# tum-vision/mem

Measured on AMD Instinct MI355X. Metric: pretrain samples/sec (ViT-B, 224^2 event voxels), higher is better.
Workload: dtype bf16; 1 GPU; MEM pretrain ViT-Base/16, 224^2 2-bin event voxels, bf16, batch 256 per GPU (BASELINE configs[1]); step = rasterize 256x30k events + event_norm + masks + ViT fwd/CE/bwd + clip + AdamW; global_batch=256, parallelism=dp1, stochastic_depth=work skipping, optimizer=AdamW as one launch in front of the next forward, last_block_mlp_rows=rows that reach the head

## Files before the change

mem_amd/csrc/misc.hip:

```cpp
#include "common.h"

namespace {

using namespace memhip;

typedef __attribute__((ext_vector_type(4))) __bf16 bf16x4;
typedef __attribute__((ext_vector_type(8))) __bf16 bf16x8;

__global__ __launch_bounds__(256) void cast_kernel(const float* __restrict__ in, __bf16* __restrict__ out,
                                                   long long n4) {
  for (long long i = (long long)blockIdx.x * 256 + threadIdx.x; i < n4; i += (long long)gridDim.x * 256) {
    const float4 v = reinterpret_cast<const float4*>(in)[i];
    bf16x4 o;
    o[0] = (__bf16)v.x; o[1] = (__bf16)v.y; o[2] = (__bf16)v.z; o[3] = (__bf16)v.w;
    reinterpret_cast<bf16x4*>(out)[i] = o;
  }
}

template <typename IN>
__global__ __launch_bounds__(256) void transpose_kernel(const IN* __restrict__ in, long long ldin, int R,
                                                        int Cc, __bf16* __restrict__ out, long long ldout,
                                                        int R_pad, float* __restrict__ cs0, int c0b, int c0e,
                                                        float* __restrict__ cs1, int c1b, int c1e) {
  __shared__ __bf16 tile[64][66];
  const int r0 = blockIdx.x * 64, c0 = blockIdx.y * 64;
  const int t = threadIdx.x;
#pragma unroll
  for (int pass = 0; pass < 2; ++pass) {
    const int rl = (t >> 3) + pass * 32, cl = (t & 7) * 8;
    const int r = r0 + rl;
#pragma unroll
    for (int k = 0; k < 8; ++k) {
      const int c = c0 + cl + k;
      __bf16 v = (__bf16)0.f;
      if (r < R && c < Cc) v = (__bf16)(float)in[(long long)r * ldin + c];
      tile[rl][cl + k] = v;
    }
  }
  __syncthreads();
#pragma unroll
  for (int pass = 0; pass < 2; ++pass) {
    const int cl = (t >> 3) + pass * 32, rl = (t & 7) * 8;
    const int c = c0 + cl;
    bf16x8 o;
    float s = 0.f;
#pragma unroll
    for (int k = 0; k < 8; ++k) { o[k] = tile[rl + k][cl]; s += (float)o[k]; }
    if (c < Cc && r0 + rl < R_pad)
      *reinterpret_cast<bf16x8*>(out + (long long)c * ldout + r0 + rl) = o;
    if (cs0 || cs1) {
      s += __shfl_xor(s, 1); s += __shfl_xor(s, 2); s += __shfl_xor(s, 4);
      if ((t & 7) == 0 && c < Cc) {
        if (cs0 && c >= c0b && c < c0e) atomicAdd(cs0 + (c - c0b), s);
        if (cs1 && c >= c1b && c < c1e) atomicAdd(cs1 + (c - c1b), s);
      }
    }
  }
}

struct TransposeDesc { const float* in; long long ldin; long long R; long long Cc; __bf16* out; long long ldout; };
__global__ __launch_bounds__(256) void transpose_cast_batched_kernel(const TransposeDesc* __restrict__ desc,
                                                                     const int* __restrict__ tile_prefix, int n) {
  __shared__ __bf16 tile[64][66];
  int mi = 0;
  while (mi + 1 < n && (int)blockIdx.x >= tile_prefix[mi + 1]) ++mi;
  const TransposeDesc d = desc[mi];
  const int local = blockIdx.x - tile_prefix[mi];
  const int R = (int)d.R, Cc = (int)d.Cc;
  const int tr = (R + 63) / 64;
  const int r0 = (local % tr) * 64, c0 = (local / tr) * 64;
  const int t = threadIdx.x;
  const int R_pad = (int)(d.ldout < (long long)tr * 64 ? d.ldout : (long long)tr * 64);
#pragma unroll
  for (int pass = 0; pass < 2; ++pass) {
    const int rl = (t >> 3) + pass * 32, cl = (t & 7) * 8;
    const int r = r0 + rl, c = c0 + cl;
    const float* src = d.in + (long long)r * d.ldin + c;
    if (r < R && c + 8 <= Cc && ((d.ldin & 3) == 0) && (((unsigned long long)d.in & 15) == 0)) {
      const float4 a = reinterpret_cast<const float4*>(src)[0], b = reinterpret_cast<const float4*>(src)[1];
      const float v[8] = {a.x, a.y, a.z, a.w, b.x, b.y, b.z, b.w};
#pragma unroll
      for (int k = 0; k < 8; ++k) tile[rl][cl + k] = (__bf16)v[k];
    } else {
#pragma unroll
      for (int k = 0; k < 8; ++k) tile[rl][cl + k] = (r < R && c + k < Cc) ? (__bf16)src[k] : (__bf16)0.f;
    }
  }
  __syncthreads();
#pragma unroll
  for (int pass = 0; pass < 2; ++pass) {
    const int cl = (t >> 3) + pass * 32, rl = (t & 7) * 8;
    const int c = c0 + cl;
    bf16x8 o;
#pragma unroll
    for (int k = 0; k < 8; ++k) o[k] = tile[rl + k][cl];
    if (c < Cc && r0 + rl < R_pad) *reinterpret_cast<bf16x8*>(d.out + (long long)c * d.ldout + r0 + rl) = o;
  }
}

__global__ __launch_bounds__(256) void im2col_kernel(const float* __restrict__ x, int B, int C, int H, int W,
                                                     int ph, int pw, __bf16* __restrict__ out) {
  const int gw = W / pw, gh = H / ph;
  const int K = C * ph * pw, K8 = K >> 3;
  const long long total = (long long)B * gh * gw * K8;
  for (long long i = (long long)blockIdx.x * 256 + threadIdx.x; i < total; i += (long long)gridDim.x * 256) {
    const int k8 = (int)(i % K8);
    const long long row = i / K8;
    const int k = k8 * 8;
    const int c = k / (ph * pw), rem = k - c * ph * pw, py = rem / pw, px = rem - py * pw;
    const int gx = (int)(row % gw);
    const long long t = row / gw;
    const int gy = (int)(t % gh), b = (int)(t / gh);
    const float* src = x + (((long long)b * C + c) * H + gy * ph + py) * W + gx * pw + px;
    const float4 a = reinterpret_cast<const float4*>(src)[0], d = reinterpret_cast<const float4*>(src)[1];
    bf16x8 o;
    o[0] = (__bf16)a.x; o[1] = (__bf16)a.y; o[2] = (__bf16)a.z; o[3] = (__bf16)a.w;
    o[4] = (__bf16)d.x; o[5] = (__bf16)d.y; o[6] = (__bf16)d.z; o[7] = (__bf16)d.w;
    reinterpret_cast<bf16x8*>(out)[i] = o;
  }
}

__global__ __launch_bounds__(256) void fill_cls_kernel(float* __restrict__ x, long long ldx, int B, int T, int D,
                                                       const float* __restrict__ cls) {
  const int b = blockIdx.x;
  for (int c = threadIdx.x; c < D; c += 256) x[(long long)b * T * ldx + c] = cls[c];
}

__global__ __launch_bounds__(256) void relpos_gather_kernel(const float* __restrict__ table,
                                                            const int* __restrict__ idx, int T, int TP, int Hh,
                                                            float* __restrict__ bias, float* __restrict__ biasT) {
  const long long total = (long long)Hh * TP * TP;
  for (long long i = (long long)blockIdx.x * 256 + threadIdx.x; i < total; i += (long long)gridDim.x * 256) {
    const int k = (int)(i % TP);
    const long long t = i / TP;
    const int q = (int)(t % TP), h = (int)(t / TP);
    float v = 0.f;
    if (q < T && k < T) v = table[(long long)idx[q * T + k] * Hh + h];
    bias[i] = v;
    if (biasT) biasT[((long long)h * TP + k) * TP + q] = v;
  }
}


__global__ __launch_bounds__(256) void gemv_acc_kernel(const __bf16* __restrict__ W, long long ldw, int N, int K,
                                                       const float* __restrict__ x, float* __restrict__ y,
                                                       float* __restrict__ x_acc, float* __restrict__ zero) {
  const int lane = threadIdx.x & 63;
  const int n = blockIdx.x * 4 + (threadIdx.x >> 6);
  if (n < N) {
    float s = 0.f;
    for (int k = lane * 8; k < K; k += 512) {
      const bf16x8 w = *reinterpret_cast<const bf16x8*>(W + (long long)n * ldw + k);
      const float4 a = *reinterpret_cast<const float4*>(x + k), b = *reinterpret_cast<const float4*>(x + k + 4);
      s += (float)w[0] * a.x + (float)w[1] * a.y + (float)w[2] * a.z + (float)w[3] * a.w + (float)w[4] * b.x +
           (float)w[5] * b.y + (float)w[6] * b.z + (float)w[7] * b.w;
    }
    for (int o = 32; o > 0; o >>= 1) s += __shfl_xor(s, o);
    if (lane == 0) y[n] += s;
  }
  if (blockIdx.x == 0) {
    for (int k = threadIdx.x; k < K; k += blockDim.x) {
      if (x_acc) x_acc[k] += x[k];
      if (zero) zero[k] = 0.f;
    }
  }
}

}

extern "C" int memhip_cast_f32_bf16(const float* in, void* out, int64_t n, memhip_stream_t stream) {
  MEMHIP_REQUIRE(n >= 0 && n % 4 == 0, "cast: n must be a multiple of 4");
  if (n == 0) return MEMHIP_OK;
  MEMHIP_REQUIRE(in && out, "cast: null pointer");
  const long long n4 = n / 4;
  int blocks = (int)((n4 + 255) / 256);
  if (blocks > 4096) blocks = 4096;
  hipLaunchKernelGGL(cast_kernel, dim3(blocks), dim3(256), 0, as_stream(stream), in, (__bf16*)out, n4);
  return check_launch("cast_f32_bf16");
}

extern "C" int memhip_transpose_cast_f32_bf16(const float* in, int64_t ldin, int R, int Cc, void* out,
                                              int64_t ldout, memhip_stream_t stream) {
  MEMHIP_REQUIRE(R > 0 && Cc > 0 && in && out, "transpose_cast: bad arguments");
  MEMHIP_REQUIRE(ldout % 8 == 0 && ldout >= R, "transpose_cast: ldout");
  const int R_pad = (int)(ldout < (int64_t)cdiv(R, 64) * 64 ? ldout : (int64_t)cdiv(R, 64) * 64);
  hipLaunchKernelGGL(transpose_kernel<float>, dim3(cdiv(R, 64), cdiv(Cc, 64)), dim3(256), 0, as_stream(stream), in,
                     (long long)ldin, R, Cc, (__bf16*)out, (long long)ldout, R_pad, (float*)nullptr, 0, 0,
                     (float*)nullptr, 0, 0);
  return check_launch("transpose_cast");
}

extern "C" int memhip_transpose_cast_batched(const void* desc, const int32_t* tile_prefix, int n, int total_tiles,
                                             memhip_stream_t stream) {
  MEMHIP_REQUIRE(n >= 0 && total_tiles >= 0, "transpose_cast_batched: bad arguments");
  if (n == 0 || total_tiles == 0) return MEMHIP_OK;
  MEMHIP_REQUIRE(desc && tile_prefix, "transpose_cast_batched: null pointer");
  static_assert(sizeof(TransposeDesc) == 48, "descriptor = 6 x 8 bytes");
  hipLaunchKernelGGL(transpose_cast_batched_kernel, dim3(total_tiles), dim3(256), 0, as_stream(stream),
                     (const TransposeDesc*)desc, tile_prefix, n);
  return check_launch("transpose_cast_batched");
}

extern "C" int memhip_transpose_bf16(const void* in, int64_t ldin, int R, int Cc, void* out, int64_t ldout,
                                     int R_pad, float* colsum0, int c0_begin, int c0_end, float* colsum1,
                                     int c1_begin, int c1_end, memhip_stream_t stream) {
  MEMHIP_REQUIRE(R >= 0 && Cc > 0 && in && out, "transpose: bad arguments");
  MEMHIP_REQUIRE(R_pad >= R && R_pad % 64 == 0 && ldout >= R_pad && ldout % 8 == 0,
                 "transpose: R_pad=%d must be a multiple of 64 and <= ldout", R_pad);
  if (R_pad == 0) return MEMHIP_OK;
  hipLaunchKernelGGL(transpose_kernel<__bf16>, dim3(R_pad / 64, cdiv(Cc, 64)), dim3(256), 0, as_stream(stream),
                     (const __bf16*)in, (long long)ldin, R, Cc, (__bf16*)out, (long long)ldout, R_pad, colsum0,
                     c0_begin, c0_end, colsum1, c1_begin, c1_end);
  return check_launch("transpose_bf16");
}

extern "C" int memhip_im2col_bf16(const float* x, int B, int C, int H, int W, int ph, int pw, void* out,
                                  memhip_stream_t stream) {
  MEMHIP_REQUIRE(B >= 0 && C > 0 && ph > 0 && pw > 0 && H % ph == 0 && W % pw == 0, "im2col: bad shape");
  MEMHIP_REQUIRE(pw % 8 == 0 && W % 4 == 0, "im2col: patch width must be a multiple of 8");
  if (B == 0) return MEMHIP_OK;
  MEMHIP_REQUIRE(x && out, "im2col: null pointer");
  const long long total = (long long)B * (H / ph) * (W / pw) * (C * ph * pw / 8);
  int blocks = (int)((total + 255) / 256);
  if (blocks > 8192) blocks = 8192;
  hipLaunchKernelGGL(im2col_kernel, dim3(blocks), dim3(256), 0, as_stream(stream), x, B, C, H, W, ph, pw,
                     (__bf16*)out);
  return check_launch("im2col");
}

__global__ __launch_bounds__(256) void copy_samples_kernel(const float* __restrict__ src, float* __restrict__ dst,
                                                           const int* __restrict__ ids, long long n_per_sample) {
  const long long base = (long long)ids[blockIdx.y] * n_per_sample;
  const float4* s4 = reinterpret_cast<const float4*>(src + base);
  float4* d4 = reinterpret_cast<float4*>(dst + base);
  for (long long i = (long long)blockIdx.x * 256 + threadIdx.x; i < n_per_sample / 4; i += (long long)gridDim.x * 256) d4[i] = s4[i];
}

extern "C" int memhip_copy_samples_f32(const float* src, float* dst, const int32_t* ids, int n, int64_t n_per_sample,
// ... 136 lines not shown
```

mem_amd/csrc/rowops.hip:

```cpp
#include "common.h"
#include "dropout.hpp"

#include <type_traits>

namespace {

using namespace memhip;

typedef __attribute__((ext_vector_type(4))) __bf16 bf16x4;
typedef __attribute__((ext_vector_type(8))) __bf16 bf16x8;

__device__ __forceinline__ float wsum(float v) {
  for (int o = 32; o > 0; o >>= 1) v += __shfl_xor(v, o);
  return v;
}
__device__ __forceinline__ float wmax(float v) {
  for (int o = 32; o > 0; o >>= 1) v = fmaxf(v, __shfl_xor(v, o));
  return v;
}

__device__ __forceinline__ float div_newton(float a, float b, float r) {
  const float q0 = a * r;
  return fmaf(fmaf(-q0, b, a), r, q0);
}

constexpr int kMaxChunks = 8;

template <bool FULL>
__device__ __forceinline__ bool chunk_ok(int i, int nch) {
  if constexpr (FULL) return true;
  else return i < nch;
}

__device__ __forceinline__ int wave_id() { return __builtin_amdgcn_readfirstlane((int)(threadIdx.x >> 6)); }

struct RowWalk {
  int r, smp, off, stride, q, rem, rps;
  __device__ __forceinline__ RowWalk(int r0, int stride_, int rps_) : r(r0), stride(stride_), rps(rps_) {
    smp = r0 / rps; off = r0 - smp * rps;
    q = stride / rps; rem = stride - q * rps;
  }
  __device__ __forceinline__ void next() {
    r += stride; smp += q; off += rem;
    if (off >= rps) { off -= rps; ++smp; }
  }
};

__device__ __forceinline__ void stage_columns(float4* dst, const float* a, const float* b, int nch) {
  for (int i = threadIdx.x; i < nch; i += 256) {
    dst[i] = reinterpret_cast<const float4*>(a)[i];
    dst[nch + i] = b ? reinterpret_cast<const float4*>(b)[i] : float4{1.f, 1.f, 1.f, 1.f};
  }
  __syncthreads();
}

__device__ __forceinline__ int opaque(int v) {
  asm volatile("" : "+v"(v));
  return v;
}

__device__ __forceinline__ float mul_rn(float a, float b) {
#pragma clang fp contract(off)
  return a * b;
}
__device__ __forceinline__ float sub_rn(float a, float b) {
#pragma clang fp contract(off)
  return a - b;
}
__device__ __forceinline__ float ln_dx(float gg, float xh, float m1, float m2) { return __fmaf_rn(-xh, m2, sub_rn(gg, m1)); }
__device__ __forceinline__ float sq2(float a, float b) { return __fmaf_rn(a, a, mul_rn(b, b)); }

template <int NCH, bool FULL>
__global__ __launch_bounds__(256) void ln_fwd_kernel(const float* __restrict__ x, long long ldx,
                                                     const int* __restrict__ row_idx, int R, int D,
                                                     const float* __restrict__ gamma,
                                                     const float* __restrict__ beta, float eps,
                                                     __bf16* __restrict__ y, long long ldy,
                                                     float* __restrict__ mean, float* __restrict__ rstd) {
  extern __shared__ float red[];
  const int lane = threadIdx.x & 63;
  const int r0 = blockIdx.x * 4 + wave_id();
  const bool act = r0 < R;
  const int r = act ? r0 : R - 1;
  const long long src = row_idx ? row_idx[r] : r;
  const float4* xr = reinterpret_cast<const float4*>(x + src * ldx);
  const int nch = D >> 2;
  float4 v[NCH];
#pragma unroll
  for (int c = 0; c < NCH; ++c) {
    const int i = lane + c * 64;
    if (chunk_ok<FULL>(i, nch)) v[c] = xr[i];
  }
  constexpr int NST = (64 * NCH + 255) / 256;
  float4 sg[NST], sb[NST];
#pragma unroll
  for (int k = 0; k < NST; ++k) {
    const int i = min((int)threadIdx.x + k * 256, nch - 1);
    sg[k] = reinterpret_cast<const float4*>(gamma)[i];
    sb[k] = reinterpret_cast<const float4*>(beta)[i];
  }
  __builtin_amdgcn_sched_barrier(0);
  float s = 0.f;
#pragma unroll
  for (int c = 0; c < NCH; ++c)
    if (chunk_ok<FULL>(lane + c * 64, nch)) s += (v[c].x + v[c].y) + (v[c].z + v[c].w);
  const float mu = wsum(s) / (float)D;
  float4* lgb = reinterpret_cast<float4*>(red);
#pragma unroll
  for (int k = 0; k < NST; ++k) {
    const int i = min((int)threadIdx.x + k * 256, nch - 1);
    lgb[i] = sg[k];
    lgb[nch + i] = sb[k];
  }
  float q = 0.f;
#pragma unroll
  for (int c = 0; c < NCH; ++c) {
    if (chunk_ok<FULL>(lane + c * 64, nch)) {
      const float a = v[c].x - mu, b = v[c].y - mu, cc = v[c].z - mu, d = v[c].w - mu;
      q += sq2(a, b) + sq2(cc, d);
    }
  }
  const float var = wsum(q) / (float)D;
  const float rs = 1.0f / sqrtf(var + eps);
  __syncthreads();
  if (!act) return;
  if (lane == 0) { mean[r] = mu; rstd[r] = rs; }
  bf16x4* yr = reinterpret_cast<bf16x4*>(y + (long long)r * ldy);
#pragma unroll
  for (int c = 0; c < NCH; ++c) {
    const int i = lane + c * 64;
    if (chunk_ok<FULL>(i, nch)) {
      const float4 g = lgb[i], b = lgb[nch + i];
      bf16x4 o;
      o[0] = (__bf16)__fmaf_rn(mul_rn(v[c].x - mu, rs), g.x, b.x);
      o[1] = (__bf16)__fmaf_rn(mul_rn(v[c].y - mu, rs), g.y, b.y);
      o[2] = (__bf16)__fmaf_rn(mul_rn(v[c].z - mu, rs), g.z, b.z);
      o[3] = (__bf16)__fmaf_rn(mul_rn(v[c].w - mu, rs), g.w, b.w);
      yr[i] = o;
    }
  }
}

__device__ __forceinline__ void vm_drain() { __builtin_amdgcn_s_waitcnt(0x0F70); }

template <int NCH, bool FULL, bool ACC>
__global__ __launch_bounds__(256) void ln_bwd_kernel(const __bf16* __restrict__ dy, long long lddy,
                                                     const float* __restrict__ x, long long ldx,
                                                     const int* __restrict__ row_idx, int R, int D,
                                                     const float* __restrict__ gamma,
                                                     const float* __restrict__ mean,
                                                     const float* __restrict__ rstd,
                                                     float* __restrict__ dres, long long lddres,
                                                     float* __restrict__ dgamma, float* __restrict__ dbeta) {
  extern __shared__ float red[];
  const int lane = threadIdx.x & 63, wave = wave_id();
  const int nch = D >> 2;
  float4 ag[NCH], ab[NCH];
#pragma unroll
  for (int c = 0; c < NCH; ++c) {
    ag[c] = float4{0, 0, 0, 0};
    ab[c] = float4{0, 0, 0, 0};
  }
  const int rstride = gridDim.x * 4;
  float4 xn[NCH], prev[NCH];
  bf16x4 dn[NCH];
  auto issue = [&](int r, long long src, int lane) {
    const float4* xr = reinterpret_cast<const float4*>(x + src * ldx);
    const bf16x4* dyr = reinterpret_cast<const bf16x4*>(dy + (long long)r * lddy);
#pragma unroll
    for (int c = 0; c < NCH; ++c) {
      const int i = lane + c * 64;
      if (chunk_ok<FULL>(i, nch)) {
        xn[c] = xr[i];
        dn[c] = dyr[i];
      }
    }
  };
  auto issue_prev = [&](long long src, int lane) {
    const float4* o = reinterpret_cast<const float4*>(dres + src * lddres);
#pragma unroll
    for (int c = 0; c < NCH; ++c) {
      const int i = lane + c * 64;
      if (chunk_ok<FULL>(i, nch)) prev[c] = o[i];
    }
  };
  int r = blockIdx.x * 4 + wave;
  long long src = 0;
  float mu = 0.f, rs = 0.f;
  if (r < R) {
    src = row_idx ? row_idx[r] : r;
    issue(r, src, lane);
    if constexpr (ACC) issue_prev(src, lane);
    mu = mean[r]; rs = rstd[r];
  }
  float4* lg = reinterpret_cast<float4*>(red);
  for (int i = threadIdx.x; i < nch; i += 256) lg[i] = reinterpret_cast<const float4*>(gamma)[i];
  __syncthreads();
  int r1 = r + rstride;
  long long src1 = 0;
  if (r1 < R) src1 = row_idx ? row_idx[r1] : r1;
  int r2 = r1 + rstride;
  vm_drain();
  while (r < R) {
    float4 xh[NCH], gg[NCH];
    float s1 = 0.f, s2 = 0.f;
    const int ol = opaque(lane);
    const float4* lgl = lg + ol;
#pragma unroll
    for (int c = 0; c < NCH; ++c) {
      const int i = lane + c * 64;
      if (chunk_ok<FULL>(i, nch)) {
        const float4 xv = xn[c];
        const bf16x4 d4 = dn[c];
        const float4 g = lgl[c * 64];
        const float d0 = (float)d4[0], d1 = (float)d4[1], d2 = (float)d4[2], d3 = (float)d4[3];
        xh[c] = float4{mul_rn(xv.x - mu, rs), mul_rn(xv.y - mu, rs), mul_rn(xv.z - mu, rs), mul_rn(xv.w - mu, rs)};
        gg[c] = float4{mul_rn(d0, g.x), mul_rn(d1, g.y), mul_rn(d2, g.z), mul_rn(d3, g.w)};
        s1 += (gg[c].x + gg[c].y) + (gg[c].z + gg[c].w);
        s2 += (mul_rn(gg[c].x, xh[c].x) + mul_rn(gg[c].y, xh[c].y)) + (mul_rn(gg[c].z, xh[c].z) + mul_rn(gg[c].w, xh[c].w));
        ag[c].x += d0 * xh[c].x; ag[c].y += d1 * xh[c].y; ag[c].z += d2 * xh[c].z; ag[c].w += d3 * xh[c].w;
// ... 243 lines not shown
  };
  int r, rin, rout;
  float mu = 0.f, rs = 0.f, km = 1.f;
  float4 xh[NCH], gg[NCH];
  bf16x4 yv[HAS_Y ? NCH : 1];
  float s1, s2;
  float4 *lg = reinterpret_cast<float4*>(red), *lgb = lg + nch;
  auto reduce_row = [&](bool has_in, int ol) {
    s1 = s2 = 0.f;
    const float4* lgl = lg + ol;
    if (has_in) {
#pragma unroll
      for (int c = 0; c < NCH; ++c) {
        if (chunk_ok<FULL>(lane + c * 64, nch)) {
          if constexpr (HAS_Y) yv[c] = yn[c];
          const float4 xv = xn[c];
          const bf16x4 d4 = dn[c];
          const float d0 = (float)d4[0], d1 = (float)d4[1], d2 = (float)d4[2], d3 = (float)d4[3];
          xh[c] = float4{mul_rn(xv.x - mu, rs), mul_rn(xv.y - mu, rs), mul_rn(xv.z - mu, rs), mul_rn(xv.w - mu, rs)};
          const float4 gmc = lgl[c * 64];
          gg[c] = float4{mul_rn(d0, gmc.x), mul_rn(d1, gmc.y), mul_rn(d2, gmc.z), mul_rn(d3, gmc.w)};
          s1 += (gg[c].x + gg[c].y) + (gg[c].z + gg[c].w);
          s2 += (mul_rn(gg[c].x, xh[c].x) + mul_rn(gg[c].y, xh[c].y)) + (mul_rn(gg[c].z, xh[c].z) + mul_rn(gg[c].w, xh[c].w));
          ag[c].x += d0 * xh[c].x; ag[c].y += d1 * xh[c].y; ag[c].z += d2 * xh[c].z; ag[c].w += d3 * xh[c].w;
          ab[c].x += d0; ab[c].y += d1; ab[c].z += d2; ab[c].w += d3;
        }
      }
    } else {
#pragma unroll
      for (int c = 0; c < NCH; ++c) {
        if (chunk_ok<FULL>(lane + c * 64, nch)) {
          if constexpr (HAS_Y) yv[c] = yn[c];
          xh[c] = gg[c] = float4{0.f, 0.f, 0.f, 0.f};
        }
      }
    }
  };
  auto store_row = [&](bool has_in, bool has_out, int ol) {
    const float m1 = wsum(s1) / (float)D, m2 = wsum(s2) / (float)D;
    float4* o = reinterpret_cast<float4*>(dres + (long long)r * lddres);
    bf16x4* orow = reinterpret_cast<bf16x4*>(dyo + (long long)(has_out ? rout : 0) * lddyo);
    const float4* lgbl = lgb + ol;
#pragma unroll
    for (int c = 0; c < NCH; ++c) {
      const int i = ol + c * 64;
      if (chunk_ok<FULL>(i, nch)) {
        float4 d{__fmaf_rn(rs, ln_dx(gg[c].x, xh[c].x, m1, m2), prev[c].x), __fmaf_rn(rs, ln_dx(gg[c].y, xh[c].y, m1, m2), prev[c].y),
                 __fmaf_rn(rs, ln_dx(gg[c].z, xh[c].z, m1, m2), prev[c].z), __fmaf_rn(rs, ln_dx(gg[c].w, xh[c].w, m1, m2), prev[c].w)};
        if (has_in) o[i] = d;
        if (!has_out) continue;
        if (rowmask || out_map) {
          d.x = div_newton(d.x * km, keep, rk); d.y = div_newton(d.y * km, keep, rk);
          d.z = div_newton(d.z * km, keep, rk); d.w = div_newton(d.w * km, keep, rk);
        }
        if constexpr (sizeof...(Drop) > 0) {
          const DropParams dp = (drop, ...);
          const unsigned kb = dropout_keep8(dp, (unsigned)(dp.row0 + r), (unsigned)(i >> 1)) >> ((i & 1) * 4);
          d.x = __fmul_rn(d.x, dropout_mul(dp, kb, 0)); d.y = __fmul_rn(d.y, dropout_mul(dp, kb, 1));
          d.z = __fmul_rn(d.z, dropout_mul(dp, kb, 2)); d.w = __fmul_rn(d.w, dropout_mul(dp, kb, 3));
        }
        if constexpr (HAS_Y) {
          bg[c].x += d.x * (float)yv[c][0]; bg[c].y += d.y * (float)yv[c][1];
          bg[c].z += d.z * (float)yv[c][2]; bg[c].w += d.w * (float)yv[c][3];
        }
        const float4 gbc = lgbl[c * 64];
        bf16x4 q;
        q[0] = (__bf16)(d.x * gbc.x); q[1] = (__bf16)(d.y * gbc.y);
        q[2] = (__bf16)(d.z * gbc.z); q[3] = (__bf16)(d.w * gbc.w);
        orow[i] = q;
        bb[c].x += (float)q[0]; bb[c].y += (float)q[1]; bb[c].z += (float)q[2]; bb[c].w += (float)q[3];
      }
    }
  };
  RowWalk w(row0, rstride, rps);
  auto find = [&](int& fr, int& frin, int& frout, int& fsmp) {
    for (;;) {
      fr = w.r; fsmp = w.smp; frin = frout = -1;
      if (fr >= R) return;
      resolve(w, frin, frout);
      w.next();
      if ((frin | frout) >= 0) return;
    }
  };
  int smp;
  find(r, rin, rout, smp);
  if (r < R) {
    issue_x(r, rin, lane); issue_y(r, lane); issue_prev(r, lane);
    mu = mean[rin]; rs = rstd[rin];
    if (rowmask) km = rowmask[smp];
  }
  stage_columns(lg, gamma, gb, nch);
  int r1, rin1, rout1, smp1;
  find(r1, rin1, rout1, smp1);
  vm_drain();
  while (r < R) {
    const int ol = opaque(lane);
    reduce_row(true, ol);
    float mu1 = 0.f, rs1 = 0.f, km1 = 1.f;
    const bool next = r1 < R;
    const int rl = next ? r1 : r, rinl = next ? rin1 : rin;
    issue_x(rl, rinl, ol); issue_y(rl, ol);
    if (next) {
      mu1 = mean[rin1]; rs1 = rstd[rin1];
      if (rowmask) km1 = rowmask[smp1];
    }
    int r2, rin2, rout2, smp2;
    find(r2, rin2, rout2, smp2);
    store_row(true, true, ol);
    __builtin_amdgcn_sched_barrier(0);
    issue_prev(rl, ol);
    r = r1; rin = rin1; rout = rout1; mu = mu1; rs = rs1; km = km1;
    r1 = r2; rin1 = rin2; rout1 = rout2; smp1 = smp2;
  }
  if (in_map || out_map) {
    for (RowWalk v(row0, rstride, rps); v.r < R; v.next()) {
      resolve(v, rin, rout);
      if ((rin >= 0) == (rout >= 0)) continue;
      r = v.r;
      const int ol = opaque(lane);
      issue_prev(r, ol); issue_y(r, ol);
      mu = rs = 0.f;
      if (rin >= 0) {
        issue_x(r, rin, ol);
        mu = mean[rin]; rs = rstd[rin];
      }
      km = rowmask ? rowmask[v.smp] : 1.f;
      reduce_row(rin >= 0, ol);
      store_row(rin >= 0, rout >= 0, ol);
    }
  }
  __syncthreads();
  float4* r0 = reinterpret_cast<float4*>(red + (size_t)wave * 4 * D);
#pragma unroll
  for (int c = 0; c < NCH; ++c) {
    const int i = lane + c * 64;
    if (chunk_ok<FULL>(i, nch)) { r0[i] = ag[c]; r0[nch + i] = ab[c]; r0[2 * nch + i] = HAS_Y ? bg[HAS_Y ? c : 0] : float4{0, 0, 0, 0}; r0[3 * nch + i] = bb[c]; }
  }
  __syncthreads();
  for (int n = threadIdx.x; n < D; n += 256) {
    float a = 0.f, b = 0.f, c2 = 0.f, d2 = 0.f;
#pragma unroll
    for (int w2 = 0; w2 < 4; ++w2) {
      const float* rw = red + (size_t)w2 * 4 * D;
      a += rw[n]; b += rw[D + n]; c2 += rw[2 * D + n]; d2 += rw[3 * D + n];
    }
    atomicAdd(dgamma + n, a);
    atomicAdd(dbeta + n, b);
    if (dgb) atomicAdd(dgb + n, c2);
    if (dbiasb) atomicAdd(dbiasb + n, d2);
  }
}


__global__ __launch_bounds__(256) void layerscale_grad_kernel(const __bf16* __restrict__ W, long long ldw,
                                                              const float* __restrict__ dW, long long lddw,
                                                              const float* __restrict__ b, const float* __restrict__ db,
                                                              const float* __restrict__ gamma, int N, int K,
                                                              float* __restrict__ dgamma) {
  __shared__ float red[4][4];
  const int lane = threadIdx.x & 63, wave = threadIdx.x >> 6;
  const int n0 = blockIdx.x * 4;
  float s[4] = {0.f, 0.f, 0.f, 0.f};
  for (int k0 = 0; k0 < K; k0 += 4096) {
#pragma unroll
    for (int c = 0; c < 4; ++c) {
      const int n = n0 + c < N ? n0 + c : N - 1;
      const __bf16* wr = W + (long long)n * ldw;
      const float* gr = dW + (long long)n * lddw;
#pragma unroll
      for (int u = 0; u < 4; ++u) {
        const int k = k0 + u * 1024 + (int)threadIdx.x * 4;
        if (k < K) {
          const bf16x4 w = *reinterpret_cast<const bf16x4*>(wr + k);
          const float4 g = *reinterpret_cast<const float4*>(gr + k);
          s[c] += (float)w[0] * g.x + (float)w[1] * g.y + (float)w[2] * g.z + (float)w[3] * g.w;
        }
      }
    }
  }
#pragma unroll
  for (int c = 0; c < 4; ++c) {
    const float t = wsum(s[c]);
    if (lane == 0) red[wave][c] = t;
  }
  __syncthreads();
  if (threadIdx.x < 4 && n0 + (int)threadIdx.x < N) {
    const int n = n0 + threadIdx.x;
    float t = (red[0][threadIdx.x] + red[1][threadIdx.x]) + (red[2][threadIdx.x] + red[3][threadIdx.x]);
    if (b && db) t += b[n] * db[n];
    const float g = gamma[n];
    dgamma[n] = g != 0.f ? t / g : 0.f;
  }
}

__global__ __launch_bounds__(256) void embed_bwd_kernel(const float* __restrict__ dx, long long lddx,
                                                        const unsigned char* __restrict__ mask, int B,
                                                        int L, int D, __bf16* __restrict__ dy,
                                                        long long lddy, float* __restrict__ dcls,
                                                        float* __restrict__ dmask) {
  constexpr int U = 7;
  for (int c = threadIdx.x * 4; c < D; c += 256 * 4) {
    float4 cls{0, 0, 0, 0}, am{0, 0, 0, 0};
    for (int b = blockIdx.x; b < B; b += gridDim.x) {
      const float* row0 = dx + (long long)b * (L + 1) * lddx + c;
      const float4 dc = *reinterpret_cast<const float4*>(row0);
      cls.x += dc.x; cls.y += dc.y; cls.z += dc.z; cls.w += dc.w;
      const unsigned char* mk = mask + (long long)b * L;
      __bf16* out = dy + (long long)b * L * lddy + c;
      int p = 0;
      for (; p + U <= L; p += U) {
        float4 d[U];
#pragma unroll
        for (int u = 0; u < U; ++u) d[u] = *reinterpret_cast<const float4*>(row0 + (long long)(1 + p + u) * lddx);
#pragma unroll
        for (int u = 0; u < U; ++u) {
          const float w = (float)mk[p + u], q = 1.0f - w;
          am.x += d[u].x * w; am.y += d[u].y * w; am.z += d[u].z * w; am.w += d[u].w * w;
          bf16x4 o;
          o[0] = (__bf16)(d[u].x * q); o[1] = (__bf16)(d[u].y * q); o[2] = (__bf16)(d[u].z * q); o[3] = (__bf16)(d[u].w * q);
          *reinterpret_cast<bf16x4*>(out + (long long)(p + u) * lddy) = o;
        }
      }
      for (; p < L; ++p) {
        const float4 d = *reinterpret_cast<const float4*>(row0 + (long long)(1 + p) * lddx);
        const float w = (float)mk[p], q = 1.0f - w;
        am.x += d.x * w; am.y += d.y * w; am.z += d.z * w; am.w += d.w * w;
        bf16x4 o;
        o[0] = (__bf16)(d.x * q); o[1] = (__bf16)(d.y * q); o[2] = (__bf16)(d.z * q); o[3] = (__bf16)(d.w * q);
        *reinterpret_cast<bf16x4*>(out + (long long)p * lddy) = o;
      }
    }
    atomicAdd(dcls + c, cls.x); atomicAdd(dcls + c + 1, cls.y);
    atomicAdd(dcls + c + 2, cls.z); atomicAdd(dcls + c + 3, cls.w);
    atomicAdd(dmask + c, am.x); atomicAdd(dmask + c + 1, am.y);
    atomicAdd(dmask + c + 2, am.z); atomicAdd(dmask + c + 3, am.w);
  }
}

template <int VPT>
__global__ __launch_bounds__(256) void ce_kernel(__bf16* __restrict__ logits, long long ld,
                                                 const long long* __restrict__ labels, int V,
                                                 float grad_scale, float* __restrict__ row_loss,
                                                 int* __restrict__ row_correct, int write_grad) {
  __shared__ float sm[4];
  __shared__ int si[4];
  __shared__ float bc[2];
  const int r = blockIdx.x, tid = threadIdx.x, lane = tid & 63, wave = tid >> 6;
  bf16x8* row = reinterpret_cast<bf16x8*>(logits + (long long)r * ld);
  const int nch = V >> 3;
  float v[VPT][8];
  float mx = -INFINITY;
  int amax = 0x7fffffff;
#pragma unroll
  for (int c = 0; c < VPT; ++c) {
    const int i = tid + c * 256;
    if (i < nch) {
      const bf16x8 t = row[i];
#pragma unroll
      for (int k = 0; k < 8; ++k) {
        v[c][k] = (float)t[k];
        if (v[c][k] > mx) { mx = v[c][k]; amax = i * 8 + k; }
      }
    }
  }
  for (int o = 32; o > 0; o >>= 1) {
    const float om = __shfl_xor(mx, o);
    const int oi = __shfl_xor(amax, o);
    if (om > mx || (om == mx && oi < amax)) { mx = om; amax = oi; }
  }
  if (lane == 0) { sm[wave] = mx; si[wave] = amax; }
  __syncthreads();
  if (tid == 0) {
    float m = sm[0]; int a = si[0];
    for (int w = 1; w < 4; ++w) if (sm[w] > m || (sm[w] == m && si[w] < a)) { m = sm[w]; a = si[w]; }
    bc[0] = m; si[0] = a;
  }
  __syncthreads();
  mx = bc[0];
  amax = si[0];
  float s = 0.f;
#pragma unroll
  for (int c = 0; c < VPT; ++c) {
    const int i = tid + c * 256;
    if (i < nch) {
#pragma unroll
      for (int k = 0; k < 8; ++k) { v[c][k] = __expf(v[c][k] - mx); s += v[c][k]; }
    }
  }
  s = wsum(s);
  __syncthreads();
  if (lane == 0) sm[wave] = s;
  __syncthreads();
  if (tid == 0) bc[1] = (sm[0] + sm[1]) + (sm[2] + sm[3]);
  __syncthreads();
  const float sum = bc[1];
  const long long lab = labels[r];
  if (tid == 0) {
    const bool lab_ok = lab >= 0 && lab < V;
    const float zl = lab_ok ? (float)logits[(long long)r * ld + lab] : __builtin_nanf("");
    row_loss[r] = (mx + __logf(sum)) - zl;
    row_correct[r] = (amax == (int)lab) ? 1 : 0;
  }
  if (write_grad) {
    const float inv = 1.0f / sum;
    __syncthreads();
#pragma unroll
    for (int c = 0; c < VPT; ++c) {
      const int i = tid + c * 256;
      if (i < nch) {
        bf16x8 o;
#pragma unroll
        for (int k = 0; k < 8; ++k) {
          float p = v[c][k] * inv;
          if ((long long)(i * 8 + k) == lab) p -= 1.0f;
          o[k] = (__bf16)(p * grad_scale);
        }
        row[i] = o;
      }
    }
  }
}

__global__ __launch_bounds__(256) void ce_reduce_kernel(const float* __restrict__ row_loss,
                                                        const int* __restrict__ row_correct, int M,
                                                        float* __restrict__ out) {
  __shared__ double sd[4];
  __shared__ int sc[4];
  double s = 0.0;
  int c = 0;
  for (int i = threadIdx.x; i < M; i += 256) { s += (double)row_loss[i]; c += row_correct[i]; }
  for (int o = 32; o > 0; o >>= 1) { s += __shfl_xor(s, o); c += __shfl_xor(c, o); }
  if ((threadIdx.x & 63) == 0) { sd[threadIdx.x >> 6] = s; sc[threadIdx.x >> 6] = c; }
  __syncthreads();
  if (threadIdx.x == 0) {
    const double t = (sd[0] + sd[1]) + (sd[2] + sd[3]);
    const int k = sc[0] + sc[1] + sc[2] + sc[3];
    out[0] = (float)(t / (double)M);
    out[1] = (float)k / (float)M;
  }
}

}

template <int MAXN, class F>
void dispatch_width(int D, F&& f) {
  const int nch = cdiv(D / 4, 64);
  const bool full = D % 256 == 0;
  const auto either = [&](auto N) { if (full) f(N, std::true_type{}); else f(N, std::false_type{}); };
  if (nch <= 1) either(std::integral_constant<int, 1>{});
  else if (nch <= 2) either(std::integral_constant<int, 2>{});
  else if (nch <= 3) either(std::integral_constant<int, 3>{});
  else if (MAXN == 4 || nch <= 4) either(std::integral_constant<int, 4>{});
  else if constexpr (MAXN == 8) {
    if (nch == 5 && full) f(std::integral_constant<int, 5>{}, std::true_type{});
    else if (nch == 8 && full) f(std::integral_constant<int, 8>{}, std::true_type{});
    else f(std::integral_constant<int, 8>{}, std::false_type{});
  }
}

extern "C" int memhip_layernorm_fwd(const float* x, int64_t ldx, const int32_t* row_idx, int R, int D,
                                    const float* gamma, const float* beta, float eps, void* y,
                                    int64_t ldy, float* mean, float* rstd, memhip_stream_t stream) {
  MEMHIP_REQUIRE(R >= 0 && D > 0 && D % 4 == 0 && D <= 64 * 4 * kMaxChunks, "layernorm_fwd: bad R=%d D=%d", R, D);
  if (R == 0) return MEMHIP_OK;
  MEMHIP_REQUIRE(x && gamma && beta && y && mean && rstd, "layernorm_fwd: null pointer");
  MEMHIP_REQUIRE(ldx % 4 == 0 && ldy % 4 == 0, "layernorm_fwd: ld must be a multiple of 4");
  dispatch_width<kMaxChunks>(D, [&](auto N, auto F) {
    hipLaunchKernelGGL((ln_fwd_kernel<decltype(N)::value, decltype(F)::value>), dim3(cdiv(R, 4)), dim3(256), (size_t)2 * D * sizeof(float), as_stream(stream),
                       x, (long long)ldx, row_idx, R, D, gamma, beta, eps, (__bf16*)y, (long long)ldy, mean, rstd);
  });
  return check_launch("layernorm_fwd");
}

extern "C" int memhip_layernorm_bwd(const void* dy, int64_t lddy, const float* x, int64_t ldx,
                                    const int32_t* row_idx, int R, int D, const float* gamma,
                                    const float* mean, const float* rstd, float* dres, int64_t lddres,
                                    int accumulate, float* dgamma, float* dbeta, memhip_stream_t stream) {
  MEMHIP_REQUIRE(R >= 0 && D > 0 && D % 4 == 0 && D <= 64 * 4 * kMaxChunks, "layernorm_bwd: bad R=%d D=%d", R, D);
  if (R == 0) return MEMHIP_OK;
  MEMHIP_REQUIRE(dy && x && gamma && mean && rstd && dres && dgamma && dbeta, "layernorm_bwd: null pointer");
  MEMHIP_REQUIRE(ldx % 4 == 0 && lddy % 4 == 0 && lddres % 4 == 0, "layernorm_bwd: ld must be a multiple of 4");
  int grid = cdiv(R, 4);
  const int cap = opt(OPT_LN_BWD_GRID) * 4 / 3;
  if (grid > cap) grid = cap;
  dispatch_width<kMaxChunks>(D, [&](auto N, auto F) {
    dispatch_bool(accumulate, [&](auto A) {
      hipLaunchKernelGGL((ln_bwd_kernel<decltype(N)::value, decltype(F)::value, decltype(A)::value>), dim3(grid), dim3(256), (size_t)8 * D * sizeof(float), as_stream(stream),
                         (const __bf16*)dy, (long long)lddy, x, (long long)ldx, row_idx, R, D, gamma, mean, rstd, dres,
                         (long long)lddres, dgamma, dbeta);
      return 0;
    });
  });
  return check_launch("layernorm_bwd");
}

template <int NCH, bool FULL, bool HAS_Y, class... Drop>
static void branch_bwd_launch(const memhip_branch_bwd_args_t& a, int grid, memhip_stream_t stream, Drop... drop) {
  const memhip_branch_t& b = a.branch;
  hipLaunchKernelGGL((branch_bwd_kernel<NCH, FULL, HAS_Y, Drop...>), dim3(grid), dim3(256), (size_t)8 * a.D * sizeof(float),
                     as_stream(stream), a.dx, (long long)a.lddx, (const __bf16*)b.y, (long long)b.ldy, b.gamma, b.rowmask,
                     b.keep_prob, b.rows_per_sample > 0 ? b.rows_per_sample : 1, a.M, a.D, (__bf16*)b.dy, (long long)b.lddy,
                     b.dgamma, b.dbias, (const int*)b.out_map, drop...);
}

extern "C" int memhip_branch_bwd(const memhip_branch_bwd_args_t* args, memhip_stream_t stream) {
  MEMHIP_REQUIRE(args, "branch_bwd: null args");
  const memhip_branch_t& b = args->branch;
  const int M = args->M, D = args->D;
  MEMHIP_REQUIRE(M >= 0 && D > 0 && D % 4 == 0, "branch_bwd: bad M=%d D=%d", M, D);
  MEMHIP_REQUIRE(!b.dropout || D % 8 == 0, "branch_bwd_drop: D=%d must be a multiple of 8", D);
  MEMHIP_REQUIRE(!b.out_map || (!b.rowmask && !b.y && b.rows_per_sample > 0), "branch_bwd: out_map excludes rowmask / y");
  if (M == 0) return MEMHIP_OK;
  MEMHIP_REQUIRE(args->dx && b.dy, "branch_bwd: null pointer");
  MEMHIP_REQUIRE(b.y || !b.dgamma, "branch_bwd: dgamma needs y (or use memhip_layerscale_grad)");
  MEMHIP_REQUIRE(args->lddx % 4 == 0 && b.ldy % 4 == 0 && b.lddy % 4 == 0, "branch_bwd: ld must be a multiple of 4");
  MEMHIP_REQUIRE(D <= 64 * 4 * kBrMaxChunks, "branch_bwd: D=%d too large", D);
  int grid = cdiv(M, 4);
  if (grid > 1024) grid = 1024;
  dispatch_width<kBrMaxChunks>(D, [&](auto N, auto F) {
    dispatch_bool(b.y, [&](auto Y) {
      if (b.dropout) branch_bwd_launch<decltype(N)::value, decltype(F)::value, decltype(Y)::value>(*args, grid, stream, drop_params(*b.dropout));
      else branch_bwd_launch<decltype(N)::value, decltype(F)::value, decltype(Y)::value>(*args, grid, stream);
      return 0;
    });
  });
  return check_launch("branch_bwd");
}

extern "C" int memhip_embed_bwd(const float* dx, int64_t lddx, const uint8_t* mask, int B, int L, int D,
                                void* dy, int64_t lddy, float* dcls, float* dmask_token,
                                memhip_stream_t stream) {
  MEMHIP_REQUIRE(B >= 0 && L > 0 && D > 0 && D % 4 == 0, "embed_bwd: bad shape");
  if (B == 0) return MEMHIP_OK;
  MEMHIP_REQUIRE(dx && mask && dy && dcls && dmask_token, "embed_bwd: null pointer");
  hipLaunchKernelGGL(embed_bwd_kernel, dim3(B < 128 ? B : 128), dim3(256), 0, as_stream(stream), dx, (long long)lddx, mask, B,
                     L, D, (__bf16*)dy, (long long)lddy, dcls, dmask_token);
  return check_launch("embed_bwd");
}

extern "C" int memhip_cross_entropy(void* logits, int64_t ld, const int64_t* labels, int M, int V,
                                    float grad_scale, float* row_loss, int32_t* row_correct,
                                    int write_grad, float* out2, memhip_stream_t stream) {
  MEMHIP_REQUIRE(M >= 0 && V > 0 && V % 8 == 0 && V <= 256 * 8 * 8, "cross_entropy: V=%d unsupported", V);
  if (M == 0) return MEMHIP_OK;
  MEMHIP_REQUIRE(logits && labels && row_loss && row_correct && out2, "cross_entropy: null pointer");
  MEMHIP_REQUIRE(ld % 8 == 0, "cross_entropy: ld must be a multiple of 8");
  hipStream_t s = as_stream(stream);
  const int nch = V / 8, vpt = cdiv(nch, 256);
  __bf16* lg = (__bf16*)logits;
  const long long* lab = (const long long*)labels;
#define CE_LAUNCH(N) hipLaunchKernelGGL(ce_kernel<N>, dim3(M), dim3(256), 0, s, lg, (long long)ld, lab, V, \
                                        grad_scale, row_loss, row_correct, write_grad)
  if (vpt <= 1) CE_LAUNCH(1);
  else if (vpt <= 2) CE_LAUNCH(2);
  else if (vpt <= 4) CE_LAUNCH(4);
  else CE_LAUNCH(8);
#undef CE_LAUNCH
  hipLaunchKernelGGL(ce_reduce_kernel, dim3(1), dim3(256), 0, s, row_loss, row_correct, M, out2);
  return check_launch("cross_entropy");
}

template <int NCH, bool FULL, bool HAS_Y, class... Drop>
static void ln_bwd_branch_launch(const memhip_ln_bwd_branch_args_t& a, int grid, memhip_stream_t stream, Drop... drop) {
  const memhip_branch_t& b = a.branch;
  hipLaunchKernelGGL((ln_bwd_branch_kernel<NCH, FULL, HAS_Y, Drop...>), dim3(grid), dim3(256), (size_t)16 * a.D * sizeof(float),
                     as_stream(stream), (const __bf16*)a.dy, (long long)a.lddy, a.x, (long long)a.ldx, a.R, a.D, a.gamma, a.mean,
                     a.rstd, a.dres, (long long)a.lddres, a.dgamma, a.dbeta, (const __bf16*)b.y, (long long)b.ldy, b.gamma,
                     b.rowmask, b.keep_prob, b.rows_per_sample > 0 ? b.rows_per_sample : 1, (__bf16*)b.dy, (long long)b.lddy,
                     b.dgamma, b.dbias, (const int*)a.in_map, (const int*)b.out_map, drop...);
}

extern "C" int memhip_layernorm_bwd_branch(const memhip_ln_bwd_branch_args_t* args, memhip_stream_t stream) {
  MEMHIP_REQUIRE(args, "layernorm_bwd_branch: null args");
  const memhip_ln_bwd_branch_args_t& a = *args;
  const memhip_branch_t& b = a.branch;
  const int R = a.R, D = a.D;
  MEMHIP_REQUIRE(R >= 0 && D > 0 && D % 4 == 0 && D <= 64 * 4 * 4, "layernorm_bwd_branch: D=%d unsupported (<= 1024)", D);
  MEMHIP_REQUIRE(!b.dropout || D % 8 == 0, "layernorm_bwd_branch_drop: D=%d must be a multiple of 8", D);
  MEMHIP_REQUIRE(!(a.in_map || b.out_map) || (!b.rowmask && !b.y && b.rows_per_sample > 0),
                 "layernorm_bwd_branch: sample maps exclude rowmask / y_branch");
  if (R == 0) return MEMHIP_OK;
  MEMHIP_REQUIRE(a.dy && a.x && a.gamma && a.mean && a.rstd && a.dres && a.dgamma && a.dbeta && b.dy,
                 "layernorm_bwd_branch: null pointer");
// ... 33 lines not shown
```

Baseline: 7659 samples/sec.

## Batch loads ahead of use in cast, transpose, layerscale-grad and CE reduce kernels

Several small memory-bound helper kernels are restructured so their global loads are issued in batches before the values are used. The cast kernel gains double-buffered prefetch with scheduling barriers. The batched transpose replaces its serial prefix search with a wave ballot and adds a fast interior path. Layerscale-grad and ce_reduce issue all their loads up front, with ce_reduce also using vector loads staged through LDS. These are auxiliary kernels in a ViT training step dominated by GEMMs and attention, so the effect on end-to-end throughput is likely small. The extra code raises register and LDS use.

New measurement: 7671 samples/sec, median of 3. Within noise of the previous version (+0.2%).

```diff
diff --git a/mem_amd/csrc/misc.hip b/mem_amd/csrc/misc.hip
--- a/mem_amd/csrc/misc.hip
+++ b/mem_amd/csrc/misc.hip
@@ -7,13 +7,51 @@
 typedef __attribute__((ext_vector_type(4))) __bf16 bf16x4;
 typedef __attribute__((ext_vector_type(8))) __bf16 bf16x8;
 
-__global__ __launch_bounds__(256) void cast_kernel(const float* __restrict__ in, __bf16* __restrict__ out,
-                                                   long long n4) {
-  for (long long i = (long long)blockIdx.x * 256 + threadIdx.x; i < n4; i += (long long)gridDim.x * 256) {
-    const float4 v = reinterpret_cast<const float4*>(in)[i];
-    bf16x4 o;
-    o[0] = (__bf16)v.x; o[1] = (__bf16)v.y; o[2] = (__bf16)v.z; o[3] = (__bf16)v.w;
-    reinterpret_cast<bf16x4*>(out)[i] = o;
+__device__ __forceinline__ void vm_drain() { __builtin_amdgcn_s_waitcnt(0x0F70); }
+
+__device__ __forceinline__ bf16x4 cast4(const float4 v) {
+  bf16x4 o;
+  o[0] = (__bf16)v.x; o[1] = (__bf16)v.y; o[2] = (__bf16)v.z; o[3] = (__bf16)v.w;
+  return o;
+}
+
+constexpr int kCastU = 2;
+__global__ __launch_bounds__(256) void cast_kernel(const float* in, __bf16* out, long long n4) {
+  const float4* in4 = reinterpret_cast<const float4*>(in);
+  bf16x4* out4 = reinterpret_cast<bf16x4*>(out);
+  const long long nfull = n4 / (kCastU * 256), stride = gridDim.x;
+  struct Tile { float4 v[kCastU]; long long t, i; };
+  const auto request = [&](Tile& k, const long long t) {
+    k.t = t;
+    k.i = t * (kCastU * 256) + threadIdx.x;
+#pragma unroll
+    for (int u = 0; u < kCastU; ++u) k.v[u] = in4[k.i + u * 256];
+  };
+  const auto trip = [&](Tile& cur, Tile& nxt) {
+    const long long tn = cur.t + stride;
+    const bool more = tn < nfull;
+    request(nxt, more ? tn : cur.t);
+    __builtin_amdgcn_sched_barrier(0);
+#pragma unroll
+    for (int u = 0; u < kCastU; ++u) out4[cur.i + u * 256] = cast4(cur.v[u]);
+    __builtin_amdgcn_sched_barrier(0);
+    return more;
+  };
+  if ((long long)blockIdx.x < nfull) {
+    Tile a, b;
+    request(a, blockIdx.x);
+    vm_drain();
+    for (;;) {
+      if (!trip(a, b)) break;
+      if (!trip(b, a)) break;
+    }
+  }
+  if (blockIdx.x == gridDim.x - 1) {
+#pragma unroll
+    for (int u = 0; u < kCastU; ++u) {
+      const long long i = nfull * (kCastU * 256) + u * 256 + threadIdx.x;
+      if (i < n4) out4[i] = cast4(in4[i]);
+    }
   }
 }
 
@@ -62,8 +100,14 @@
 __global__ __launch_bounds__(256) void transpose_cast_batched_kernel(const TransposeDesc* __restrict__ desc,
                                                                      const int* __restrict__ tile_prefix, int n) {
   __shared__ __bf16 tile[64][66];
+  const int lane = threadIdx.x & 63;
   int mi = 0;
-  while (mi + 1 < n && (int)blockIdx.x >= tile_prefix[mi + 1]) ++mi;
+  for (int j0 = 1; j0 < n; j0 += 64) {
+    const int j = j0 + lane;
+    const int first = tile_prefix[j < n ? j : n - 1];
+    mi += __popcll(__ballot(j < n && (int)blockIdx.x >= first));
+  }
+  mi = __builtin_amdgcn_readfirstlane(mi);
   const TransposeDesc d = desc[mi];
   const int local = blockIdx.x - tile_prefix[mi];
   const int R = (int)d.R, Cc = (int)d.Cc;
@@ -71,19 +115,35 @@
   const int r0 = (local % tr) * 64, c0 = (local / tr) * 64;
   const int t = threadIdx.x;
   const int R_pad = (int)(d.ldout < (long long)tr * 64 ? d.ldout : (long long)tr * 64);
-#pragma unroll
-  for (int pass = 0; pass < 2; ++pass) {
-    const int rl = (t >> 3) + pass * 32, cl = (t & 7) * 8;
-    const int r = r0 + rl, c = c0 + cl;
-    const float* src = d.in + (long long)r * d.ldin + c;
-    if (r < R && c + 8 <= Cc && ((d.ldin & 3) == 0) && (((unsigned long long)d.in & 15) == 0)) {
-      const float4 a = reinterpret_cast<const float4*>(src)[0], b = reinterpret_cast<const float4*>(src)[1];
-      const float v[8] = {a.x, a.y, a.z, a.w, b.x, b.y, b.z, b.w};
-#pragma unroll
-      for (int k = 0; k < 8; ++k) tile[rl][cl + k] = (__bf16)v[k];
-    } else {
-#pragma unroll
-      for (int k = 0; k < 8; ++k) tile[rl][cl + k] = (r < R && c + k < Cc) ? (__bf16)src[k] : (__bf16)0.f;
+  const bool aligned = ((d.ldin & 3) == 0) && (((unsigned long long)d.in & 15) == 0);
+  const bool interior = r0 + 64 <= R && c0 + 64 <= Cc;
+  const auto put8 = [&](const int rl, const int cl, const float4 a, const float4 b) {
+    const float v[8] = {a.x, a.y, a.z, a.w, b.x, b.y, b.z, b.w};
+#pragma unroll
+    for (int k = 0; k < 8; ++k) tile[rl][cl + k] = (__bf16)v[k];
+  };
+  if (aligned && interior) {
+    float4 a[2], b[2];
+#pragma unroll
+    for (int pass = 0; pass < 2; ++pass) {
+      const float* src = d.in + (long long)(r0 + (t >> 3) + pass * 32) * d.ldin + c0 + (t & 7) * 8;
+      a[pass] = reinterpret_cast<const float4*>(src)[0];
+      b[pass] = reinterpret_cast<const float4*>(src)[1];
+    }
+#pragma unroll
+    for (int pass = 0; pass < 2; ++pass) put8((t >> 3) + pass * 32, (t & 7) * 8, a[pass], b[pass]);
+  } else {
+#pragma unroll
+    for (int pass = 0; pass < 2; ++pass) {
+      const int rl = (t >> 3) + pass * 32, cl = (t & 7) * 8;
+      const int r = r0 + rl, c = c0 + cl;
+      const float* src = d.in + (long long)r * d.ldin + c;
+      if (aligned && r < R && c + 8 <= Cc) {
+        put8(rl, cl, reinterpret_cast<const float4*>(src)[0], reinterpret_cast<const float4*>(src)[1]);
+      } else {
+#pragma unroll
+        for (int k = 0; k < 8; ++k) tile[rl][cl + k] = (r < R && c + k < Cc) ? (__bf16)src[k] : (__bf16)0.f;
+      }
     }
   }
   __syncthreads();
diff --git a/mem_amd/csrc/rowops.hip b/mem_amd/csrc/rowops.hip
--- a/mem_amd/csrc/rowops.hip
+++ b/mem_amd/csrc/rowops.hip
@@ -66,6 +66,10 @@
 __device__ __forceinline__ float sub_rn(float a, float b) {
 #pragma clang fp contract(off)
   return a - b;
+}
+__device__ __forceinline__ float dot4_rn(const bf16x4 w, const float4 g) {
+#pragma clang fp contract(off)
+  return (float)w[0] * g.x + (float)w[1] * g.y + (float)w[2] * g.z + (float)w[3] * g.w;
 }
 __device__ __forceinline__ float ln_dx(float gg, float xh, float m1, float m2) { return __fmaf_rn(-xh, m2, sub_rn(gg, m1)); }
 __device__ __forceinline__ float sq2(float a, float b) { return __fmaf_rn(a, a, mul_rn(b, b)); }
@@ -615,7 +619,7 @@
 }
 
 
-__global__ __launch_bounds__(256) void layerscale_grad_kernel(const __bf16* __restrict__ W, long long ldw,
+__global__ __launch_bounds__(256) __attribute__((amdgpu_waves_per_eu(1, 4))) void layerscale_grad_kernel(const __bf16* __restrict__ W, long long ldw,
                                                               const float* __restrict__ dW, long long lddw,
                                                               const float* __restrict__ b, const float* __restrict__ db,
                                                               const float* __restrict__ gamma, int N, int K,
@@ -625,6 +629,8 @@
   const int n0 = blockIdx.x * 4;
   float s[4] = {0.f, 0.f, 0.f, 0.f};
   for (int k0 = 0; k0 < K; k0 += 4096) {
+    bf16x4 w[4][4];
+    float4 g[4][4];
 #pragma unroll
     for (int c = 0; c < 4; ++c) {
       const int n = n0 + c < N ? n0 + c : N - 1;
@@ -633,13 +639,18 @@
 #pragma unroll
       for (int u = 0; u < 4; ++u) {
         const int k = k0 + u * 1024 + (int)threadIdx.x * 4;
-        if (k < K) {
-          const bf16x4 w = *reinterpret_cast<const bf16x4*>(wr + k);
-          const float4 g = *reinterpret_cast<const float4*>(gr + k);
-          s[c] += (float)w[0] * g.x + (float)w[1] * g.y + (float)w[2] * g.z + (float)w[3] * g.w;
-        }
-      }
-    }
+        const int kc = k < K ? k : 0;
+        w[c][u] = *reinterpret_cast<const bf16x4*>(wr + kc);
+        g[c][u] = *reinterpret_cast<const float4*>(gr + kc);
+      }
+    }
+#pragma unroll
+    for (int c = 0; c < 4; ++c)
+#pragma unroll
+      for (int u = 0; u < 4; ++u) {
+        const float t = s[c] + dot4_rn(w[c][u], g[c][u]);
+        s[c] = k0 + u * 1024 + (int)threadIdx.x * 4 < K ? t : s[c];
+      }
   }
 #pragma unroll
   for (int c = 0; c < 4; ++c) {
@@ -784,14 +795,55 @@
   }
 }
 
+constexpr int kCeU = 8;
 __global__ __launch_bounds__(256) void ce_reduce_kernel(const float* __restrict__ row_loss,
                                                         const int* __restrict__ row_correct, int M,
                                                         float* __restrict__ out) {
+  __shared__ float rows[kCeU * 1024];
   __shared__ double sd[4];
   __shared__ int sc[4];
   double s = 0.0;
   int c = 0;
-  for (int i = threadIdx.x; i < M; i += 256) { s += (double)row_loss[i]; c += row_correct[i]; }
+  const int tid = threadIdx.x;
+  const bool aligned = ((((unsigned long long)row_loss) | ((unsigned long long)row_correct)) & 15ull) == 0;
+  const int tiles = aligned ? M / (kCeU * 1024) : 0;
+  for (int t = 0; t < tiles; ++t) {
+    const float4* l4 = reinterpret_cast<const float4*>(row_loss + (long long)t * (kCeU * 1024));
+    const int4* c4 = reinterpret_cast<const int4*>(row_correct + (long long)t * (kCeU * 1024));
+    float4 l[kCeU];
+    int4 k[kCeU];
+#pragma unroll
+    for (int u = 0; u < kCeU; ++u) {
+      l[u] = l4[u * 256 + tid];
+      k[u] = c4[u * 256 + tid];
+    }
+#pragma unroll
+    for (int u = 0; u < kCeU; ++u) {
+      reinterpret_cast<float4*>(rows)[u * 256 + tid] = l[u];
+      c += (k[u].x + k[u].y) + (k[u].z + k[u].w);
+    }
+    __syncthreads();
+#pragma unroll
+    for (int j = 0; j < kCeU * 4; ++j) s += (double)rows[j * 256 + tid];
+    __syncthreads();
+  }
+  for (int base = tiles * (kCeU * 1024); base < M; base += kCeU * 256) {
+    float l[kCeU];
+    int k[kCeU];
+#pragma unroll
+    for (int u = 0; u < kCeU; ++u) {
+      const int i = base + u * 256 + tid;
+      l[u] = row_loss[i < M ? i : M - 1];
+      k[u] = row_correct[i < M ? i : M - 1];
+    }
+#pragma unroll
+    for (int u = 0; u < kCeU; ++u) {
+      const bool ok = base + u * 256 + tid < M;
+      const double t = s + (double)l[u];
+      s = ok ? t : s;
+      c += ok ? k[u] : 0;
+    }
+  }
   for (int o = 32; o > 0; o >>= 1) { s += __shfl_xor(s, o); c += __shfl_xor(c, o); }
   if ((threadIdx.x & 63) == 0) { sd[threadIdx.x >> 6] = s; sc[threadIdx.x >> 6] = c; }
   __syncthreads();
```
